# nagadomi/nunif

Measured on NVIDIA H100. Metric: waifu2x_input_megapixels_per_sec, higher is better.
Workload: dtype f16

## Files before the change

nunif_b200/csrc/swin_attention_mma.cu:

```cuda
#include "common.cuh"
#include "gemm_wgmma.cuh"
#include "swin_kernels.h"
#include "tmap.h"

namespace nb200 {

extern int g_tune[16];

namespace {
constexpr int WS = 6, WTOK = 36, WPAD = 48, HEADS = 6;
constexpr const char* SHIFT_ONE_AXIS_MSG =
    "shifted window attention needs H and W both equal to the 6-token window or both larger (torchvision drops the shift per "
    "axis; these kernels shift both axes or neither)";
}

constexpr int NKT = 5;

template <int D>
struct AttnCtx {
    __half* sq;
    const int* sreg;
    const float4* bf;
    const __half* kbase[NKT];
    const __half* vbase[3];
    int hc, g, t4;
    float scale;
    bool boundary;
};

template <int D, int LD, bool LAST, int BNT = 6>
__device__ __forceinline__ void attn_mtile(const AttnCtx<D>& cx, int mt) {
    constexpr uint32_t ONES = 0x3C003C00u;
    constexpr int HL = LAST ? 1 : 2;
    const int g = cx.g, t4 = cx.t4, hc = cx.hc;
    const int row0 = min(mt * 16 + g, WTOK - 1), row1 = min(mt * 16 + g + 8, WTOK - 1);
    float s[NKT][4];
#pragma unroll
    for (int nt = 0; nt < NKT; ++nt)
#pragma unroll
        for (int r = 0; r < 4; ++r) s[nt][r] = 0.f;
#pragma unroll
    for (int kt = 0; kt < D / 16; ++kt) {
        uint32_t a[4];
        const __half* p0 = cx.sq + row0 * LD + hc + kt * 16 + 2 * t4;
        const __half* p1 = cx.sq + row1 * LD + hc + kt * 16 + 2 * t4;
        a[0] = *reinterpret_cast<const uint32_t*>(p0);
        a[1] = *reinterpret_cast<const uint32_t*>(p1);
        a[2] = *reinterpret_cast<const uint32_t*>(p0 + 8);
        a[3] = *reinterpret_cast<const uint32_t*>(p1 + 8);
#pragma unroll
        for (int nt = 0; nt < NKT; ++nt) {
            const __half* pk = cx.kbase[nt] + kt * 16;
            mma16816(s[nt], a, *reinterpret_cast<const uint32_t*>(pk), *reinterpret_cast<const uint32_t*>(pk + 8));
        }
    }
#pragma unroll
    for (int nt = 0; nt < NKT; ++nt) {
        const float4 bv = BNT == 6 ? __ldg(cx.bf + (mt * 6 + nt) * 32) : cx.bf[(mt * BNT + nt) * 32];
        s[nt][0] = fmaf(s[nt][0], cx.scale, bv.x);
        s[nt][1] = fmaf(s[nt][1], cx.scale, bv.y);
        if (!LAST) {
            s[nt][2] = fmaf(s[nt][2], cx.scale, bv.z);
            s[nt][3] = fmaf(s[nt][3], cx.scale, bv.w);
        }
    }
    if (cx.boundary) {
        const int q0 = cx.sreg[row0], q1 = cx.sreg[row1];
#pragma unroll
        for (int nt = 0; nt < NKT; ++nt)
#pragma unroll
            for (int e = 0; e < 2; ++e) {
                const int cr = cx.sreg[min(nt * 8 + 2 * t4 + e, WTOK - 1)];
                if (cr != q0) s[nt][e] += -100.0f * 1.4426950408889634f;
                if (!LAST && cr != q1) s[nt][2 + e] += -100.0f * 1.4426950408889634f;
            }
    }
#pragma unroll
    for (int hlf = 0; hlf < HL; ++hlf) {
        float mx = -1e30f;
#pragma unroll
        for (int nt = 0; nt < NKT; ++nt) mx = fmaxf(mx, fmaxf(s[nt][2 * hlf], s[nt][2 * hlf + 1]));
        mx = fmaxf(mx, __shfl_xor_sync(0xffffffffu, mx, 1));
        mx = fmaxf(mx, __shfl_xor_sync(0xffffffffu, mx, 2));
#pragma unroll
        for (int nt = 0; nt < NKT; ++nt)
#pragma unroll
            for (int e = 0; e < 2; ++e) {
                s[nt][2 * hlf + e] = ex2(s[nt][2 * hlf + e] - mx);
            }
    }
    if (LAST) {
#pragma unroll
        for (int nt = 0; nt < NKT; ++nt) s[nt][2] = s[nt][3] = 0.f;
    }
    float o[D / 8][4], osum[4] = {0.f, 0.f, 0.f, 0.f};
#pragma unroll
    for (int nt = 0; nt < D / 8; ++nt)
#pragma unroll
        for (int r = 0; r < 4; ++r) o[nt][r] = 0.f;
#pragma unroll
    for (int kt = 0; kt < 2; ++kt) {
        uint32_t a[4];
        a[0] = pack_half2(s[2 * kt][0], s[2 * kt][1]);
        a[1] = pack_half2(s[2 * kt][2], s[2 * kt][3]);
        a[2] = pack_half2(s[2 * kt + 1][0], s[2 * kt + 1][1]);
        a[3] = pack_half2(s[2 * kt + 1][2], s[2 * kt + 1][3]);
        mma16816(osum, a, ONES, ONES);
#pragma unroll
        for (int nt = 0; nt < D / 8; ++nt) {
            uint32_t b[2];
            ldmatrix_x2_trans(b, smem_u32(cx.vbase[kt] + nt * 8));
            mma16816(o[nt], a, b[0], b[1]);
        }
    }
    {
        const uint32_t a0 = pack_half2(s[4][0], s[4][1]), a1 = pack_half2(s[4][2], s[4][3]);
        mma1688(osum, a0, a1, ONES);
#pragma unroll
        for (int nt = 0; nt < D / 8; ++nt) {
            mma1688(o[nt], a0, a1, ldmatrix_x1_trans(smem_u32(cx.vbase[2] + nt * 8)));
        }
    }
    const float inv0 = __fdividef(1.f, osum[0]);
    const float inv1 = LAST ? 0.f : __fdividef(1.f, osum[2]);
    __syncwarp();
    const int r0 = mt * 16 + g, r1 = r0 + 8;
#pragma unroll
    for (int nt = 0; nt < D / 8; ++nt) {
        if (!LAST || r0 < WTOK) *reinterpret_cast<uint32_t*>(cx.sq + r0 * LD + hc + nt * 8 + 2 * t4) = pack_half2(o[nt][0] * inv0, o[nt][1] * inv0);
        if (!LAST) *reinterpret_cast<uint32_t*>(cx.sq + r1 * LD + hc + nt * 8 + 2 * t4) = pack_half2(o[nt][2] * inv1, o[nt][3] * inv1);
    }
}

template <int D>
__global__ void __launch_bounds__(192, D == 16 ? 6 : 4) window_attention_mma_kernel(const __half* __restrict__ qkv, const float4* __restrict__ bias_frag,
                                                                   __half* __restrict__ out, int H, int W, int shift,
                                                                   size_t plane) {
    if (threadIdx.x == 0) NB_PDL_TRIGGER();
    constexpr int C = D * HEADS;
    constexpr int LD = C + 8;
    extern __shared__ __align__(16) unsigned char smem_raw[];
    __half* sq = reinterpret_cast<__half*>(smem_raw);
    __half* sk = sq + WTOK * LD;
    __half* sv = sk + WTOK * LD;
    int* stok = reinterpret_cast<int*>(sv + WTOK * LD);
    int* sreg = stok + WTOK;
    const int nww = W / WS;
    const int wx = blockIdx.x % nww, wy = blockIdx.x / nww, b = blockIdx.y;
    const int tid = threadIdx.x;
    if (tid < WPAD) {
        int reg = -1;
        if (tid < WTOK) {
            const int ry = wy * WS + tid / WS, rx = wx * WS + tid % WS;
            const int y = (ry + shift) % H, x = (rx + shift) % W;
            stok[tid] = (b * H + y) * W + x;
            int hr = 0, wr = 0;
            if (shift > 0) {
                hr = ry < H - WS ? 0 : (ry < H - shift ? 1 : 2);
                wr = rx < W - WS ? 0 : (rx < W - shift ? 1 : 2);
            }
            reg = hr * 3 + wr;
        }
        sreg[tid] = reg;
    }
    __syncthreads();
    constexpr int VPT = C / 8;
    constexpr int RG = 192 / VPT;
    const int vv = tid % VPT, rg = tid / VPT;
    for (int t = rg; t < WTOK; t += RG) {
        const __half* src = qkv + (size_t)stok[t] * C + vv * 8;
        __half* dst = sq + t * LD + vv * 8;
        cp_async16(dst, src);
        cp_async16(dst + WTOK * LD, src + plane);
        cp_async16(dst + 2 * WTOK * LD, src + 2 * plane);
    }
    cp_async_commit();
    cp_async_wait<0>();
    __syncthreads();

    const int head = tid >> 5, lane = tid & 31, g = lane >> 2, t4 = lane & 3;
    const int hc = head * D;
    const float scale = ((D == 16) ? 0.25f : 0.17677669529663687f) * 1.4426950408889634f;
    const bool boundary = shift > 0 && (wy == gridDim.x / nww - 1 || wx == nww - 1);
    const float4* bf = bias_frag + (size_t)head * (3 * 6 * 32) + lane;
    AttnCtx<D> cx;
    cx.sq = sq; cx.sreg = sreg; cx.bf = bf; cx.hc = hc; cx.g = g; cx.t4 = t4; cx.scale = scale; cx.boundary = boundary;
#pragma unroll
    for (int nt = 0; nt < NKT; ++nt) cx.kbase[nt] = sk + min(nt * 8 + g, WTOK - 1) * LD + hc + 2 * t4;
    cx.vbase[0] = sv + (lane & 15) * LD + hc;
    cx.vbase[1] = sv + (16 + (lane & 15)) * LD + hc;
    cx.vbase[2] = sv + min(32 + (lane & 7), WTOK - 1) * LD + hc;
#pragma unroll 1
    for (int mt = 0; mt < 2; ++mt) attn_mtile<D, LD, false>(cx, mt);
    attn_mtile<D, LD, true>(cx, 2);
    __syncthreads();
    for (int t = rg; t < WTOK; t += RG)
        *reinterpret_cast<uint4*>(out + (size_t)stok[t] * C + vv * 8) = *reinterpret_cast<const uint4*>(sq + t * LD + vv * 8);
}

__global__ void build_bias_frag_kernel(const float* __restrict__ table, float4* __restrict__ frag) {
    const int i = blockIdx.x * blockDim.x + threadIdx.x;
    if (i >= HEADS * 3 * 6 * 32) return;
    const int lane = i & 31, nt = (i >> 5) % 6, mt = (i / (32 * 6)) % 3, head = i / (32 * 6 * 3);
    const int g = lane >> 2, t4 = lane & 3;
    float v[4];
#pragma unroll
    for (int r = 0; r < 4; ++r) {
        const int row = mt * 16 + g + 8 * (r >> 1), col = nt * 8 + 2 * t4 + (r & 1);
        if (col >= WTOK) v[r] = -1e30f;
        else if (row >= WTOK) v[r] = 0.f;
        else {
            const int qy = row / WS, qx = row % WS, ky = col / WS, kx = col % WS;
            v[r] = 1.4426950408889634f * table[((qy - ky + WS - 1) * (2 * WS - 1) + (qx - kx + WS - 1)) * HEADS + head];
        }
    }
    frag[i] = make_float4(v[0], v[1], v[2], v[3]);
}

int build_bias_frag(cudaStream_t st, const float* table, float* frag) {
    build_bias_frag_kernel<<<(HEADS * 3 * 6 * 32 + 255) / 256, 256, 0, st>>>(table, reinterpret_cast<float4*>(frag));
    NB_LAUNCHED();
    return 0;
}

template <int D>
static size_t attn_smem_bytes() {
    constexpr int C = D * HEADS, LD = C + 8;
    return (size_t)3 * WTOK * LD * 2 + (WTOK + WPAD) * 4 + 16;
}

static int check_window_geometry(const char* func, bool fused, int H, int W, int C, int* shift) {
    auto refuse = [&](const std::string& msg) { return fail(std::string(func) + ": " + msg); };
    if (H % WS != 0 || W % WS != 0) return refuse("feature map must be a multiple of the 6x6 window");
    if (C != 96 && C != 192) return refuse(std::string(fused ? "fused " : "") + "window attention supports C=96 (d=16) and C=192 (d=32)");
    if (*shift != 0 && (H == WS) != (W == WS)) return refuse(SHIFT_ONE_AXIS_MSG);
    if (WS >= H) *shift = 0;
    return 0;
}

int window_attention(cudaStream_t st, const __half* qkv, const float* bias_frag_f, __half* out, int B, int H, int W, int C,
                     int shift, size_t plane) {
    const float4* bias_table = reinterpret_cast<const float4*>(bias_frag_f);
    if (check_window_geometry(__func__, false, H, W, C, &shift)) return 1;
    dim3 grid((H / WS) * (W / WS), B);
    ProfScope ps(st, PC_ATTN, (double)B * H * W * C * 4 * 2, (double)B * H * W * C * 3 * 2, (double)B * H * W * C * 2);
    if (C == 96) {
        const int want = g_tune[6] > 0 ? g_tune[6] : 72;
        if (ensure_dyn_smem((const void*)window_attention_mma_kernel<16>, attn_smem_bytes<16>(), want)) return 1;
        window_attention_mma_kernel<16><<<grid, 192, attn_smem_bytes<16>(), st>>>(qkv, bias_table, out, H, W, shift, plane);
    } else {
        const int want = g_tune[6] > 0 ? g_tune[6] : 86;
        if (ensure_dyn_smem((const void*)window_attention_mma_kernel<32>, attn_smem_bytes<32>(), want)) return 1;
        window_attention_mma_kernel<32><<<grid, 192, attn_smem_bytes<32>(), st>>>(qkv, bias_table, out, H, W, shift, plane);
    }
    NB_LAUNCHED();
    return 0;
}


constexpr int FA_ROWS = 128, FA_WIN = 3, FA_SLOT = 96 * 64, FA_KPS = 3, FA_STAGES = 4;
constexpr int FA_MMA_THREADS = GEMM_CONSUMER_THREADS, FA_PRODUCER_WARP = FA_MMA_THREADS / 32, FA_ATTN_WARPS = 11;
constexpr int FA_THREADS = FA_MMA_THREADS + 32 + 32 * FA_ATTN_WARPS;
constexpr int FA_LD = 32 + 8;
constexpr int FA_CHUNK_BYTES = FA_WIN * 3 * WTOK * FA_LD * 2;
constexpr int FA_STAGE = FA_KPS * FA_SLOT;

template <int C>
struct FaCfg {
    static constexpr int X_BYTES = FA_ROWS * C * 2;
    static constexpr bool SBF = C == 96;
    static constexpr int SBF_BYTES = SBF ? HEADS * 3 * NKT * 32 * 16 : 0;
    static constexpr int SBF_OFF = 2 * X_BYTES + FA_STAGES * FA_STAGE + 2 * FA_CHUNK_BYTES + 4 * WPAD * 4 + (2 * FA_STAGES + 8) * 8 +
                                   3 * C * 4;
    static constexpr int SMEM = SBF_OFF + SBF_BYTES + 1024;
    static_assert(SBF_OFF % 16 == 0, "float4 bias fragments");
    static_assert(SMEM <= 232448, "over the 227 KB opt-in shared memory of an H100 CTA");
};

__device__ __forceinline__ int fa_token(int b, int wy, int wx, int t, int H, int W, int shift) {
    int y = wy * WS + t / WS + shift, xx = wx * WS + t % WS + shift;
    if (y >= H) y -= H;
    if (xx >= W) xx -= W;
    return (b * H + y) * W + xx;
}

template <int C>
__global__ void __launch_bounds__(FA_THREADS, 1) swin_attn_fused_kernel(const __grid_constant__ CUtensorMap wmap,
                                                                        const __half* __restrict__ x, const float* __restrict__ bqkv,
                                                                        const float4* __restrict__ bias_frag, __half* __restrict__ out,
                                                                        int H, int W, int shift, int nwin) {
    using Cfg = FaCfg<C>;
    constexpr int D = C / HEADS, KB = C / 32, NCH = C / 32, HPC = 32 / D;
    constexpr int IPC = 3 * FA_WIN * HPC, IPT = NCH * IPC;
    constexpr int SPC = KB / FA_KPS;
    constexpr int VPR = C / 8;
    static_assert(KB % FA_KPS == 0, "a ring stage holds FA_KPS K-blocks of one chunk");
    static_assert(FA_WIN == 3, "the gather selects among 3 windows");
    extern __shared__ uint8_t smem_dyn[];
    uint8_t* smem = smem_dyn + ((1024u - (smem_u32(smem_dyn) & 1023u)) & 1023u);
    uint8_t* sx = smem;
    uint8_t* ring = smem + 2 * Cfg::X_BYTES;
    __half* schunk = reinterpret_cast<__half*>(ring + FA_STAGES * FA_STAGE);
    int* sreg = reinterpret_cast<int*>(reinterpret_cast<uint8_t*>(schunk) + 2 * FA_CHUNK_BYTES);
    uint64_t* full = reinterpret_cast<uint64_t*>(sreg + 4 * WPAD);
    uint64_t* empty = full + FA_STAGES;
    uint64_t* afull = empty + FA_STAGES;
    uint64_t* aempty = afull + 2;
    uint64_t* cfull = aempty + 2;
    uint64_t* cempty = cfull + 2;
    float* sbias = reinterpret_cast<float*>(cempty + 2);
    float4* sbf = reinterpret_cast<float4*>(smem + Cfg::SBF_OFF);
    const int tid = threadIdx.x, warp = tid >> 5, lane = tid & 31;
    const int nww = W / WS, nwy = H / WS;
    const int ntiles = (nwin + FA_WIN - 1) / FA_WIN;
    const int ntl = (ntiles - (int)blockIdx.x + (int)gridDim.x - 1) / (int)gridDim.x;

    if (tid < 4 * WPAD) {
        const int p = tid / WPAD, t = tid % WPAD;
        int reg = -1;
        if (t < WTOK) {
            const int hr = (p & 2) ? (t / WS < WS - shift ? 1 : 2) : 0;
            const int wr = (p & 1) ? (t % WS < WS - shift ? 1 : 2) : 0;
            reg = hr * 3 + wr;
        }
        sreg[tid] = reg;
    }
    for (int i = tid; i < 3 * C; i += FA_THREADS) sbias[i] = bqkv[i];
    if (Cfg::SBF)
        for (int i = tid; i < HEADS * 3 * NKT * 32; i += FA_THREADS)
            sbf[i] = __ldg(bias_frag + ((i >> 5) / NKT * 6 + (i >> 5) % NKT) * 32 + (i & 31));
    for (int i = tid; i < 2 * (FA_ROWS - FA_WIN * WTOK) * VPR; i += FA_THREADS) {
        const int bsel = i / ((FA_ROWS - FA_WIN * WTOK) * VPR), j = i % ((FA_ROWS - FA_WIN * WTOK) * VPR);
        const int r = FA_WIN * WTOK + j / VPR, u = j % VPR;
        *reinterpret_cast<uint4*>(sx + bsel * Cfg::X_BYTES + (u >> 2) * (FA_ROWS * 64) + stage_off<32>(r, u & 3)) =
            make_uint4(0u, 0u, 0u, 0u);
    }
    if (tid == FA_MMA_THREADS) {
        tma_prefetch_desc(&wmap);
        for (int s = 0; s < FA_STAGES; ++s) {
            mbar_init(&full[s], 1);
            mbar_init(&empty[s], 2);
        }
        for (int b = 0; b < 2; ++b) {
            mbar_init(&afull[b], 32 * FA_ATTN_WARPS);
            mbar_init(&aempty[b], 2);
            mbar_init(&cfull[b], FA_MMA_THREADS / 32);
            mbar_init(&cempty[b], IPC);
        }
        fence_barrier_init();
    }
    fence_async_smem();
    __syncthreads();
    if (tid == 0) NB_PDL_TRIGGER();

    if (warp == FA_PRODUCER_WARP) {
        if (elect_one()) {
            int q = 0;
#pragma unroll 1
            for (int k = 0; k < ntl; ++k) {
#pragma unroll 1
                for (int i = 0; i < NCH * SPC; ++i, ++q) {
                    const int s = q % FA_STAGES, c = i / SPC, kb0 = (i % SPC) * FA_KPS;
                    mbar_wait(&empty[s], ((q / FA_STAGES) & 1) ^ 1);
                    mbar_expect_tx(&full[s], FA_STAGE);
#pragma unroll
                    for (int kk = 0; kk < FA_KPS; ++kk)
#pragma unroll
                        for (int m = 0; m < 3; ++m)
                            tma_load_2d(&wmap, &full[s], ring + s * FA_STAGE + kk * FA_SLOT + m * 32 * 64, (kb0 + kk) * 32, m * C + 32 * c);
                }
            }
        }
        return;
    }

    const float scale = ((D == 16) ? 0.25f : 0.17677669529663687f) * 1.4426950408889634f;
    const int g = lane >> 2, t4 = lane & 3;
    if (warp > FA_PRODUCER_WARP) {
        const int aw = warp - FA_PRODUCER_WARP - 1;
        auto gather = [&](int tile, uint8_t* sa) {
            int wb[FA_WIN], wwy[FA_WIN], wwx[FA_WIN];
#pragma unroll
            for (int w = 0; w < FA_WIN; ++w) {
                const int gw = tile * FA_WIN + w, b = gw / (nww * nwy), rw = gw - b * (nww * nwy);
                wb[w] = gw < nwin ? b : -1;
                wwy[w] = rw / nww;
                wwx[w] = rw - wwy[w] * nww;
            }
            for (int i = aw * 32 + lane; i < FA_WIN * WTOK * VPR; i += 32 * FA_ATTN_WARPS) {
                const int r = i / VPR, u = i % VPR, w = r / WTOK;
                const int b = w == 0 ? wb[0] : (w == 1 ? wb[1] : wb[2]);
                const int wy = w == 0 ? wwy[0] : (w == 1 ? wwy[1] : wwy[2]), wx = w == 0 ? wwx[0] : (w == 1 ? wwx[1] : wwx[2]);
                uint8_t* dst = sa + (u >> 2) * (FA_ROWS * 64) + stage_off<32>(r, u & 3);
                if (b >= 0) cp_async16(dst, x + (size_t)fa_token(b, wy, wx, r - w * WTOK, H, W, shift) * C + u * 8);
                else *reinterpret_cast<uint4*>(dst) = make_uint4(0u, 0u, 0u, 0u);
            }
            cp_async_commit();
        };
        auto gathered = [&](int kt) {
            cp_async_wait<0>();
            fence_async_smem();
            mbar_arrive(&afull[kt & 1]);
        };
        gather(blockIdx.x, sx);
        gathered(0);
        int kcur = -1, nth = 0;
#pragma unroll 1
        for (int n = aw; n < ntl * IPT; n += FA_ATTN_WARPS) {
            const int gc = n / IPC, item = n - gc * IPC, c = gc % NCH;
            const int kt = n / IPT, tile = blockIdx.x + kt * gridDim.x;
            mbar_wait(&cfull[gc & 1], (gc >> 1) & 1);
            if (kt != kcur) {
                kcur = kt;
                nth = 0;
            }
            if (kt + 1 < ntl && nth == 0) {
                mbar_wait(&aempty[(kt + 1) & 1], (((kt + 1) >> 1) & 1) ^ 1);
                gather(tile + gridDim.x, sx + ((kt + 1) & 1) * Cfg::X_BYTES);
            }
            if (kt + 1 < ntl && nth == 1) gathered(kt + 1);
            ++nth;
            const int mt = item / (FA_WIN * HPC), pr = item - mt * (FA_WIN * HPC), w = pr / HPC, hh = pr - w * HPC;
            const int gw = tile * FA_WIN + w;
            if (gw < nwin) {
                const int b = gw / (nww * nwy), r = gw % (nww * nwy), wy = r / nww, wx = r % nww, head = c * HPC + hh;
                const bool lrow = wy == nwy - 1, lcol = wx == nww - 1;
                __half* sq = schunk + (gc & 1) * (FA_CHUNK_BYTES / 2) + w * 3 * WTOK * FA_LD;
                __half* sk = sq + WTOK * FA_LD;
                __half* sv = sk + WTOK * FA_LD;
                AttnCtx<D> cx;
                cx.sq = sq; cx.sreg = sreg + (2 * lrow + lcol) * WPAD;
                cx.bf = Cfg::SBF ? sbf + head * (3 * NKT * 32) + lane : bias_frag + (size_t)head * (3 * 6 * 32) + lane;
                cx.hc = hh * D; cx.g = g; cx.t4 = t4; cx.scale = scale;
                cx.boundary = shift > 0 && (lrow || lcol);
#pragma unroll
                for (int nt = 0; nt < NKT; ++nt) cx.kbase[nt] = sk + min(nt * 8 + g, WTOK - 1) * FA_LD + cx.hc + 2 * t4;
                cx.vbase[0] = sv + (lane & 15) * FA_LD + cx.hc;
                cx.vbase[1] = sv + (16 + (lane & 15)) * FA_LD + cx.hc;
                cx.vbase[2] = sv + min(32 + (lane & 7), WTOK - 1) * FA_LD + cx.hc;
                constexpr int BNT = Cfg::SBF ? NKT : 6;
                if (mt < 2) attn_mtile<D, FA_LD, false, BNT>(cx, mt);
                else attn_mtile<D, FA_LD, true, BNT>(cx, 2);
                __syncwarp();
                const int nrow = mt < 2 ? 16 : WTOK - 32;
                for (int e = lane; e < nrow * (D / 8); e += 32) {
                    const int tk = 16 * mt + e / (D / 8), u = e % (D / 8);
                    *reinterpret_cast<uint4*>(out + (size_t)fa_token(b, wy, wx, tk, H, W, shift) * C + head * D + u * 8) =
                        *reinterpret_cast<const uint4*>(sq + tk * FA_LD + cx.hc + u * 8);
                }
            }
            __syncwarp();
            if (lane == 0) mbar_arrive(&cempty[gc & 1]);
        }
        return;
    }

    const int wg = tid >> 7, t = tid & 127;
    const int row0 = wg * 64 + (t >> 5) * 16 + ((t & 31) >> 2);
    const int cq = 2 * (t & 3);
    int q = 0, gc = 0;
#pragma unroll 1
    for (int k = 0; k < ntl; ++k) {
        mbar_wait(&afull[k & 1], (k >> 1) & 1);
        const uint32_t a_base = smem_u32(sx + (k & 1) * Cfg::X_BYTES) + wg * 64 * 64;
#pragma unroll 1
        for (int c = 0; c < NCH; ++c, ++gc) {
            float acc[48];
#pragma unroll
            for (int j = 0; j < 48; ++j) acc[j] = 0.f;
#pragma unroll 1
            for (int j = 0; j < SPC; ++j, ++q) {
                const int s = q % FA_STAGES;
                mbar_wait(&full[s], (q / FA_STAGES) & 1);
                wgmma_fence();
#pragma unroll
                for (int kk = 0; kk < FA_KPS; ++kk) {
                    const uint32_t a = a_base + (j * FA_KPS + kk) * (FA_ROWS * 64), bb = smem_u32(ring + s * FA_STAGE + kk * FA_SLOT);
                    wgmma_f16<96>(acc, make_kmajor_desc<64>(a), make_kmajor_desc<64>(bb), 1u);
                    wgmma_f16<96>(acc, make_kmajor_desc<64>(a + 32), make_kmajor_desc<64>(bb + 32), 1u);
                }
                wgmma_commit();
                wgmma_wait<1>();
                if (j > 0 && t == 0) mbar_arrive(&empty[(q - 1) % FA_STAGES]);
            }
            wgmma_wait<0>();
            if (t == 0) {
                mbar_arrive(&empty[(q - 1) % FA_STAGES]);
                if (c == NCH - 1) mbar_arrive(&aempty[k & 1]);
            }
            wgmma_fence_operands(acc);
            mbar_wait(&cempty[gc & 1], ((gc >> 1) & 1) ^ 1);
            __half* sqkv = schunk + (gc & 1) * (FA_CHUNK_BYTES / 2);
#pragma unroll
            for (int j = 0; j < 12; ++j) {
                const int m = j >> 2, col = 8 * (j & 3) + cq;
                const float2 bq = *reinterpret_cast<const float2*>(sbias + m * C + 32 * c + col);
#pragma unroll
                for (int i = 0; i < 2; ++i) {
                    const int r = row0 + 8 * i;
                    if (r < FA_WIN * WTOK) {
                        const int w = r / WTOK, tk = r - w * WTOK;
                        *reinterpret_cast<__half2*>(sqkv + ((w * 3 + m) * WTOK + tk) * FA_LD + col) =
                            __floats2half2_rn(acc[4 * j + 2 * i] + bq.x, acc[4 * j + 2 * i + 1] + bq.y);
                    }
                }
            }
            __syncwarp();
            if (lane == 0) mbar_arrive(&cfull[gc & 1]);
        }
    }
}

int swin_attn_fused(cudaStream_t st, const __half* x, const __half* wqkv, const float* bqkv, const float* bias_frag_f, __half* att,
                    int B, int H, int W, int C, int shift) {
    NB_CHECK(x && wqkv && bqkv && bias_frag_f && att, "null pointer");
    if (check_window_geometry(__func__, true, H, W, C, &shift)) return 1;
    const long long nwin = (long long)B * (H / WS) * (W / WS);
    NB_CHECK(nwin > 0 && nwin < (1LL << 31), "window count out of range");
    CUtensorMap wmap;
    const cuuint64_t dims[2] = {(cuuint64_t)C, (cuuint64_t)(3 * C)};
    const cuuint64_t strides[1] = {(cuuint64_t)C * 2};
    const cuuint32_t box[2] = {32, 32};
    if (encode(&wmap, wqkv, 2, dims, strides, box, 64)) return 1;
    const double T = (double)B * H * W;
    ProfScope ps(st, PC_FUSED_ATTN, T * 3.0 * C * C * 2 + T * C * 36 * 4, T * C * 2, T * C * 2);
    const long long ntiles = (nwin + FA_WIN - 1) / FA_WIN;
    long long grid = std::min<long long>(ntiles, device_sm_count());
    if (g_tune[11] > 0) grid = std::min<long long>(grid, g_tune[11]);
    if (rec_on()) rec_launch("swin_attn", {{"B", B}, {"H", H}, {"W", W}, {"C", C}, {"shift", shift}});
    const float4* bf = reinterpret_cast<const float4*>(bias_frag_f);
    if (C == 96) {
        if (ensure_dyn_smem((const void*)swin_attn_fused_kernel<96>, FaCfg<96>::SMEM)) return 1;
        swin_attn_fused_kernel<96><<<(unsigned)grid, FA_THREADS, FaCfg<96>::SMEM, st>>>(wmap, x, bqkv, bf, att, H, W, shift, (int)nwin);
    } else {
        if (ensure_dyn_smem((const void*)swin_attn_fused_kernel<192>, FaCfg<192>::SMEM)) return 1;
        swin_attn_fused_kernel<192><<<(unsigned)grid, FA_THREADS, FaCfg<192>::SMEM, st>>>(wmap, x, bqkv, bf, att, H, W, shift, (int)nwin);
    }
    NB_LAUNCHED();
    return 0;
}

template <typename F>
static int with_bias_frag(void* stream, const float* table, F call) {
    cudaStream_t st = (cudaStream_t)stream;
    float* frag = nullptr;
    NB_CUDA(cudaMallocAsync((void**)&frag, BIAS_FRAG_FLOATS * sizeof(float), st));
    int rc = build_bias_frag(st, table, frag);
    if (!rc) rc = call(st, frag);
    cudaFreeAsync(frag, st);
    return rc;
}

}

using namespace nb200;

extern "C" int nb200_window_attention_f16(const void* qkv, const float* bias_table, void* out, int B, int H, int W, int C,
                                          int heads, int shift, void* stream) {
    NB_CHECK(qkv && bias_table && out, "null pointer");
    NB_CHECK(heads == 6, "only 6 heads are supported");
    return with_bias_frag(stream, bias_table, [&](cudaStream_t st, const float* frag) {
        return window_attention(st, (const __half*)qkv, frag, (__half*)out, B, H, W, C, shift, (size_t)B * H * W * C);
    });
}

extern "C" int nb200_swin_attn_fused_f16(const void* x, const void* wqkv, const float* bqkv, const float* bias_table, void* att,
                                         int B, int H, int W, int C, int shift, void* stream) {
    NB_CHECK(bias_table, "null pointer");
    return with_bias_frag(stream, bias_table, [&](cudaStream_t st, const float* frag) {
        return swin_attn_fused(st, (const __half*)x, (const __half*)wqkv, bqkv, frag, (__half*)att, B, H, W, C, shift);
    });
}
```

Baseline: 80.19.

## Rebalance fused Swin attention warp roles: one MMA warpgroup and triple chunk buffers for C=96

```diff
diff --git a/nunif_b200/csrc/swin_attention_mma.cu b/nunif_b200/csrc/swin_attention_mma.cu
--- a/nunif_b200/csrc/swin_attention_mma.cu
+++ b/nunif_b200/csrc/swin_attention_mma.cu
@@ -258,19 +258,21 @@
 }
 
 
-constexpr int FA_ROWS = 128, FA_WIN = 3, FA_SLOT = 96 * 64, FA_KPS = 3, FA_STAGES = 4;
-constexpr int FA_MMA_THREADS = GEMM_CONSUMER_THREADS, FA_PRODUCER_WARP = FA_MMA_THREADS / 32, FA_ATTN_WARPS = 11;
-constexpr int FA_THREADS = FA_MMA_THREADS + 32 + 32 * FA_ATTN_WARPS;
+constexpr int FA_ROWS = 128, FA_WIN = 3, FA_SLOT = 96 * 64, FA_KPS = 3;
+constexpr int FA_WARPS = 20, FA_THREADS = 32 * FA_WARPS;
 constexpr int FA_LD = 32 + 8;
 constexpr int FA_CHUNK_BYTES = FA_WIN * 3 * WTOK * FA_LD * 2;
 constexpr int FA_STAGE = FA_KPS * FA_SLOT;
 
 template <int C>
 struct FaCfg {
+    static constexpr int MMA_WG = C == 96 ? 1 : 2;
+    static constexpr int MMA_THREADS = 128 * MMA_WG, PRODUCER_WARP = MMA_THREADS / 32, ATTN_WARPS = FA_WARPS - PRODUCER_WARP - 1;
+    static constexpr int STAGES = C == 96 ? 3 : 4, NBUF = C == 96 ? 3 : 2;
     static constexpr int X_BYTES = FA_ROWS * C * 2;
     static constexpr bool SBF = C == 96;
     static constexpr int SBF_BYTES = SBF ? HEADS * 3 * NKT * 32 * 16 : 0;
-    static constexpr int SBF_OFF = 2 * X_BYTES + FA_STAGES * FA_STAGE + 2 * FA_CHUNK_BYTES + 4 * WPAD * 4 + (2 * FA_STAGES + 8) * 8 +
+    static constexpr int SBF_OFF = 2 * X_BYTES + STAGES * FA_STAGE + NBUF * FA_CHUNK_BYTES + 4 * WPAD * 4 + (2 * STAGES + 4 + 2 * NBUF) * 8 +
                                    3 * C * 4;
     static constexpr int SMEM = SBF_OFF + SBF_BYTES + 1024;
     static_assert(SBF_OFF % 16 == 0, "float4 bias fragments");
@@ -296,19 +298,22 @@
     constexpr int VPR = C / 8;
     static_assert(KB % FA_KPS == 0, "a ring stage holds FA_KPS K-blocks of one chunk");
     static_assert(FA_WIN == 3, "the gather selects among 3 windows");
+    constexpr int STG = Cfg::STAGES, NBUF = Cfg::NBUF;
+    auto cbuf = [](int u) { return (int)((unsigned)u % NBUF); };
+    auto cpar = [](int u) { return (int)(((unsigned)u / NBUF) & 1u); };
     extern __shared__ uint8_t smem_dyn[];
     uint8_t* smem = smem_dyn + ((1024u - (smem_u32(smem_dyn) & 1023u)) & 1023u);
     uint8_t* sx = smem;
     uint8_t* ring = smem + 2 * Cfg::X_BYTES;
-    __half* schunk = reinterpret_cast<__half*>(ring + FA_STAGES * FA_STAGE);
-    int* sreg = reinterpret_cast<int*>(reinterpret_cast<uint8_t*>(schunk) + 2 * FA_CHUNK_BYTES);
+    __half* schunk = reinterpret_cast<__half*>(ring + STG * FA_STAGE);
+    int* sreg = reinterpret_cast<int*>(reinterpret_cast<uint8_t*>(schunk) + NBUF * FA_CHUNK_BYTES);
     uint64_t* full = reinterpret_cast<uint64_t*>(sreg + 4 * WPAD);
-    uint64_t* empty = full + FA_STAGES;
-    uint64_t* afull = empty + FA_STAGES;
+    uint64_t* empty = full + STG;
+    uint64_t* afull = empty + STG;
     uint64_t* aempty = afull + 2;
     uint64_t* cfull = aempty + 2;
-    uint64_t* cempty = cfull + 2;
-    float* sbias = reinterpret_cast<float*>(cempty + 2);
+    uint64_t* cempty = cfull + NBUF;
+    float* sbias = reinterpret_cast<float*>(cempty + NBUF);
     float4* sbf = reinterpret_cast<float4*>(smem + Cfg::SBF_OFF);
     const int tid = threadIdx.x, warp = tid >> 5, lane = tid & 31;
     const int nww = W / WS, nwy = H / WS;
@@ -335,16 +340,18 @@
         *reinterpret_cast<uint4*>(sx + bsel * Cfg::X_BYTES + (u >> 2) * (FA_ROWS * 64) + stage_off<32>(r, u & 3)) =
             make_uint4(0u, 0u, 0u, 0u);
     }
-    if (tid == FA_MMA_THREADS) {
+    if (tid == Cfg::MMA_THREADS) {
         tma_prefetch_desc(&wmap);
-        for (int s = 0; s < FA_STAGES; ++s) {
+        for (int s = 0; s < STG; ++s) {
             mbar_init(&full[s], 1);
-            mbar_init(&empty[s], 2);
+            mbar_init(&empty[s], Cfg::MMA_WG);
         }
         for (int b = 0; b < 2; ++b) {
-            mbar_init(&afull[b], 32 * FA_ATTN_WARPS);
-            mbar_init(&aempty[b], 2);
-            mbar_init(&cfull[b], FA_MMA_THREADS / 32);
+            mbar_init(&afull[b], 32 * Cfg::ATTN_WARPS);
+            mbar_init(&aempty[b], Cfg::MMA_WG);
+        }
+        for (int b = 0; b < NBUF; ++b) {
+            mbar_init(&cfull[b], Cfg::MMA_THREADS / 32);
             mbar_init(&cempty[b], IPC);
         }
         fence_barrier_init();
@@ -353,15 +360,15 @@
     __syncthreads();
     if (tid == 0) NB_PDL_TRIGGER();
 
-    if (warp == FA_PRODUCER_WARP) {
+    if (warp == Cfg::PRODUCER_WARP) {
         if (elect_one()) {
             int q = 0;
 #pragma unroll 1
             for (int k = 0; k < ntl; ++k) {
 #pragma unroll 1
                 for (int i = 0; i < NCH * SPC; ++i, ++q) {
-                    const int s = q % FA_STAGES, c = i / SPC, kb0 = (i % SPC) * FA_KPS;
-                    mbar_wait(&empty[s], ((q / FA_STAGES) & 1) ^ 1);
+                    const int s = q % STG, c = i / SPC, kb0 = (i % SPC) * FA_KPS;
+                    mbar_wait(&empty[s], ((q / STG) & 1) ^ 1);
                     mbar_expect_tx(&full[s], FA_STAGE);
 #pragma unroll
                     for (int kk = 0; kk < FA_KPS; ++kk)
@@ -376,8 +383,9 @@
 
     const float scale = ((D == 16) ? 0.25f : 0.17677669529663687f) * 1.4426950408889634f;
     const int g = lane >> 2, t4 = lane & 3;
-    if (warp > FA_PRODUCER_WARP) {
-        const int aw = warp - FA_PRODUCER_WARP - 1;
+    if (warp > Cfg::PRODUCER_WARP) {
+        constexpr int AWARPS = Cfg::ATTN_WARPS;
+        const int aw = warp - Cfg::PRODUCER_WARP - 1;
         auto gather = [&](int tile, uint8_t* sa) {
             int wb[FA_WIN], wwy[FA_WIN], wwx[FA_WIN];
 #pragma unroll
@@ -387,7 +395,7 @@
                 wwy[w] = rw / nww;
                 wwx[w] = rw - wwy[w] * nww;
             }
-            for (int i = aw * 32 + lane; i < FA_WIN * WTOK * VPR; i += 32 * FA_ATTN_WARPS) {
+            for (int i = aw * 32 + lane; i < FA_WIN * WTOK * VPR; i += 32 * AWARPS) {
                 const int r = i / VPR, u = i % VPR, w = r / WTOK;
                 const int b = w == 0 ? wb[0] : (w == 1 ? wb[1] : wb[2]);
                 const int wy = w == 0 ? wwy[0] : (w == 1 ? wwy[1] : wwy[2]), wx = w == 0 ? wwx[0] : (w == 1 ? wwx[1] : wwx[2]);
@@ -406,10 +414,10 @@
         gathered(0);
         int kcur = -1, nth = 0;
 #pragma unroll 1
-        for (int n = aw; n < ntl * IPT; n += FA_ATTN_WARPS) {
+        for (int n = aw; n < ntl * IPT; n += AWARPS) {
             const int gc = n / IPC, item = n - gc * IPC, c = gc % NCH;
             const int kt = n / IPT, tile = blockIdx.x + kt * gridDim.x;
-            mbar_wait(&cfull[gc & 1], (gc >> 1) & 1);
+            mbar_wait(&cfull[cbuf(gc)], cpar(gc));
             if (kt != kcur) {
                 kcur = kt;
                 nth = 0;
@@ -425,7 +433,7 @@
             if (gw < nwin) {
                 const int b = gw / (nww * nwy), r = gw % (nww * nwy), wy = r / nww, wx = r % nww, head = c * HPC + hh;
                 const bool lrow = wy == nwy - 1, lcol = wx == nww - 1;
-                __half* sq = schunk + (gc & 1) * (FA_CHUNK_BYTES / 2) + w * 3 * WTOK * FA_LD;
+                __half* sq = schunk + cbuf(gc) * (FA_CHUNK_BYTES / 2) + w * 3 * WTOK * FA_LD;
                 __half* sk = sq + WTOK * FA_LD;
                 __half* sv = sk + WTOK * FA_LD;
                 AttnCtx<D> cx;
@@ -450,63 +458,104 @@
                 }
             }
             __syncwarp();
-            if (lane == 0) mbar_arrive(&cempty[gc & 1]);
+            if (lane == 0) mbar_arrive(&cempty[cbuf(gc)]);
         }
         return;
     }
 
     const int wg = tid >> 7, t = tid & 127;
-    const int row0 = wg * 64 + (t >> 5) * 16 + ((t & 31) >> 2);
     const int cq = 2 * (t & 3);
+    auto epilogue = [&](const float (&acc)[48], int row0, int c, __half* sqkv) {
+#pragma unroll
+        for (int j = 0; j < 12; ++j) {
+            const int m = j >> 2, col = 8 * (j & 3) + cq;
+            const float2 bq = *reinterpret_cast<const float2*>(sbias + m * C + 32 * c + col);
+#pragma unroll
+            for (int i = 0; i < 2; ++i) {
+                const int r = row0 + 8 * i;
+                if (r < FA_WIN * WTOK) {
+                    const int w = r / WTOK, tk = r - w * WTOK;
+                    *reinterpret_cast<__half2*>(sqkv + ((w * 3 + m) * WTOK + tk) * FA_LD + col) =
+                        __floats2half2_rn(acc[4 * j + 2 * i] + bq.x, acc[4 * j + 2 * i + 1] + bq.y);
+                }
+            }
+        }
+    };
     int q = 0, gc = 0;
-#pragma unroll 1
-    for (int k = 0; k < ntl; ++k) {
-        mbar_wait(&afull[k & 1], (k >> 1) & 1);
-        const uint32_t a_base = smem_u32(sx + (k & 1) * Cfg::X_BYTES) + wg * 64 * 64;
-#pragma unroll 1
-        for (int c = 0; c < NCH; ++c, ++gc) {
-            float acc[48];
-#pragma unroll
-            for (int j = 0; j < 48; ++j) acc[j] = 0.f;
-#pragma unroll 1
-            for (int j = 0; j < SPC; ++j, ++q) {
-                const int s = q % FA_STAGES;
-                mbar_wait(&full[s], (q / FA_STAGES) & 1);
-                wgmma_fence();
-#pragma unroll
-                for (int kk = 0; kk < FA_KPS; ++kk) {
-                    const uint32_t a = a_base + (j * FA_KPS + kk) * (FA_ROWS * 64), bb = smem_u32(ring + s * FA_STAGE + kk * FA_SLOT);
-                    wgmma_f16<96>(acc, make_kmajor_desc<64>(a), make_kmajor_desc<64>(bb), 1u);
-                    wgmma_f16<96>(acc, make_kmajor_desc<64>(a + 32), make_kmajor_desc<64>(bb + 32), 1u);
+    if constexpr (Cfg::MMA_WG == 2) {
+        const int row0 = wg * 64 + (t >> 5) * 16 + ((t & 31) >> 2);
+#pragma unroll 1
+        for (int k = 0; k < ntl; ++k) {
+            mbar_wait(&afull[k & 1], (k >> 1) & 1);
+            const uint32_t a_base = smem_u32(sx + (k & 1) * Cfg::X_BYTES) + wg * 64 * 64;
+#pragma unroll 1
+            for (int c = 0; c < NCH; ++c, ++gc) {
+                float acc[48];
+#pragma unroll
+                for (int j = 0; j < 48; ++j) acc[j] = 0.f;
+#pragma unroll 1
+                for (int j = 0; j < SPC; ++j, ++q) {
+                    const int s = q % STG;
+                    mbar_wait(&full[s], (q / STG) & 1);
+                    wgmma_fence();
+#pragma unroll
+                    for (int kk = 0; kk < FA_KPS; ++kk) {
+                        const uint32_t a = a_base + (j * FA_KPS + kk) * (FA_ROWS * 64), bb = smem_u32(ring + s * FA_STAGE + kk * FA_SLOT);
+                        wgmma_f16<96>(acc, make_kmajor_desc<64>(a), make_kmajor_desc<64>(bb), 1u);
+                        wgmma_f16<96>(acc, make_kmajor_desc<64>(a + 32), make_kmajor_desc<64>(bb + 32), 1u);
+                    }
+                    wgmma_commit();
+                    wgmma_wait<1>();
+                    if (j > 0 && t == 0) mbar_arrive(&empty[(q - 1) % STG]);
                 }
-                wgmma_commit();
-                wgmma_wait<1>();
-                if (j > 0 && t == 0) mbar_arrive(&empty[(q - 1) % FA_STAGES]);
-            }
-            wgmma_wait<0>();
-            if (t == 0) {
-                mbar_arrive(&empty[(q - 1) % FA_STAGES]);
-                if (c == NCH - 1) mbar_arrive(&aempty[k & 1]);
-            }
-            wgmma_fence_operands(acc);
-            mbar_wait(&cempty[gc & 1], ((gc >> 1) & 1) ^ 1);
-            __half* sqkv = schunk + (gc & 1) * (FA_CHUNK_BYTES / 2);
-#pragma unroll
-            for (int j = 0; j < 12; ++j) {
-                const int m = j >> 2, col = 8 * (j & 3) + cq;
-                const float2 bq = *reinterpret_cast<const float2*>(sbias + m * C + 32 * c + col);
-#pragma unroll
-                for (int i = 0; i < 2; ++i) {
-                    const int r = row0 + 8 * i;
-                    if (r < FA_WIN * WTOK) {
-                        const int w = r / WTOK, tk = r - w * WTOK;
-                        *reinterpret_cast<__half2*>(sqkv + ((w * 3 + m) * WTOK + tk) * FA_LD + col) =
-                            __floats2half2_rn(acc[4 * j + 2 * i] + bq.x, acc[4 * j + 2 * i + 1] + bq.y);
+                wgmma_wait<0>();
+                if (t == 0) {
+                    mbar_arrive(&empty[(q - 1) % STG]);
+                    if (c == NCH - 1) mbar_arrive(&aempty[k & 1]);
+                }
+                wgmma_fence_operands(acc);
+                mbar_wait(&cempty[cbuf(gc)], cpar(gc) ^ 1);
+                epilogue(acc, row0, c, schunk + cbuf(gc) * (FA_CHUNK_BYTES / 2));
+                __syncwarp();
+                if (lane == 0) mbar_arrive(&cfull[cbuf(gc)]);
+            }
+        }
+    } else {
+        static_assert(SPC == 1, "both halves of a chunk read one ring stage");
+#pragma unroll 1
+        for (int k = 0; k < ntl; ++k) {
+            mbar_wait(&afull[k & 1], (k >> 1) & 1);
+            const uint32_t a_base = smem_u32(sx + (k & 1) * Cfg::X_BYTES);
+#pragma unroll 1
+            for (int c = 0; c < NCH; ++c, ++gc, ++q) {
+                const int s = q % STG;
+                mbar_wait(&full[s], (q / STG) & 1);
+                __half* sqkv = schunk + cbuf(gc) * (FA_CHUNK_BYTES / 2);
+#pragma unroll
+                for (int h = 0; h < 2; ++h) {
+                    float acc[48];
+#pragma unroll
+                    for (int j = 0; j < 48; ++j) acc[j] = 0.f;
+                    wgmma_fence();
+#pragma unroll
+                    for (int kk = 0; kk < FA_KPS; ++kk) {
+                        const uint32_t a = a_base + h * 64 * 64 + kk * (FA_ROWS * 64), bb = smem_u32(ring + s * FA_STAGE + kk * FA_SLOT);
+                        wgmma_f16<96>(acc, make_kmajor_desc<64>(a), make_kmajor_desc<64>(bb), 1u);
+                        wgmma_f16<96>(acc, make_kmajor_desc<64>(a + 32), make_kmajor_desc<64>(bb + 32), 1u);
                     }
+                    wgmma_commit();
+                    wgmma_wait<0>();
+                    if (h == 1 && t == 0) {
+                        mbar_arrive(&empty[s]);
+                        if (c == NCH - 1) mbar_arrive(&aempty[k & 1]);
+                    }
+                    wgmma_fence_operands(acc);
+                    if (h == 0) mbar_wait(&cempty[cbuf(gc)], cpar(gc) ^ 1);
+                    epilogue(acc, h * 64 + (t >> 5) * 16 + ((t & 31) >> 2), c, sqkv);
                 }
-            }
-            __syncwarp();
-            if (lane == 0) mbar_arrive(&cfull[gc & 1]);
+                __syncwarp();
+                if (lane == 0) mbar_arrive(&cfull[cbuf(gc)]);
+            }
         }
     }
 }
```

New measurement: 80.83, median of 6. About the same (+0.8%).
